# naturerobots/mesh_navigation

Measured on AMD Instinct MI355X. Metric: plans/sec (Dijkstra makePlan device path incl. computeVectorMap, 1M-vertex mesh), higher is better.
Workload: dtype f32

## Files before the change

### mesh_navigation_amd/csrc/mnav_tb_build.h

```cpp
#pragma once
#include <algorithm>
#include <cmath>
#include <cstdint>
#include <cstring>
#include <numeric>
#include <stdexcept>
#include <vector>

#include "mnav_build.h"

namespace mnav {

struct TbExp { uint32_t u, soff, sl, off; };

struct TbTile {
  uint32_t soff;
  uint32_t sl;
  uint32_t nv;
  uint32_t nh;
  uint32_t sweep_off;
  uint32_t sweep_chunks;
  uint32_t pre_off, pre_chunks;
  uint32_t post_off, post_chunks;
  uint32_t exp_off, exp_n;
  uint32_t v0;
  uint32_t goff;
  uint32_t ovf_off, ovf_n;
};
static_assert(sizeof(TbTile) == 64, "TbTile is read as one 64-byte scalar load");

constexpr uint32_t kTbChunk = 64;
constexpr uint32_t kTbBlock = 16;
constexpr uint32_t kTbBlocksPerChunk = 4;
constexpr uint32_t kTbGhostEdges = 5;
constexpr uint32_t kTbGhostEnd = 1u << 4;
constexpr uint32_t kTbTileEnd = 1u << 6;
constexpr uint32_t kTbOrderShift = 12;
constexpr uint32_t kTbInfBits = 0x7f800000u;
constexpr uint32_t kTbDirty = 0x80000000u;

constexpr uint32_t kTbFinSlots = 8;
constexpr uint16_t kTbFinNone = 0xFFFFu;
struct TbFinOvf { uint32_t y, src, wsrc, pad; };

struct TbvExp { uint32_t rows, soff, sl, off, n, pad[3]; };
static_assert(sizeof(TbvExp) == 32, "read as two 16-byte loads");

struct HostTb {
  std::vector<uint16_t> fin_src; std::vector<uint32_t> fin_wsrc; std::vector<TbFinOvf> fin_ovf;
  std::vector<uint32_t> ghost_gid;
  uint32_t T = 0, ntiles = 0, V = 0;
  uint64_t S = 0;
  uint32_t max_nh = 0, max_sl = 0;
  std::vector<TbTile> tiles;
  std::vector<uint32_t> stream;
  std::vector<uint32_t> wsrc;
  std::vector<uint32_t> vstream, vwsrc;
  std::vector<uint32_t> vtile;
  std::vector<TbvExp> vexps;
  std::vector<uint32_t> vgroups;
  std::vector<TbExp> exps;
  std::vector<uint32_t> verts;
  std::vector<uint32_t> vert_tile, vert_local;
};

namespace detail {
inline void tb_bisect(std::vector<uint32_t>& ids, size_t lo, size_t hi, size_t k, const float* xyz, uint32_t T, std::vector<uint32_t>& cuts)
{
  const size_t n = hi - lo;
  if (k <= 1) { cuts.push_back((uint32_t)hi); return; }
  float mn[3] = { INFINITY, INFINITY, INFINITY }, mx[3] = { -INFINITY, -INFINITY, -INFINITY };
  for (size_t i = lo; i < hi; ++i)
    for (int q = 0; q < 3; ++q) { const float x = xyz[3 * (size_t)ids[i] + q]; mn[q] = std::min(mn[q], x); mx[q] = std::max(mx[q], x); }
  int ax = 0;
  for (int q = 1; q < 3; ++q) if (mx[q] - mn[q] > mx[ax] - mn[ax]) ax = q;
  auto less = [&](uint32_t a, uint32_t b) {
    const float xa = xyz[3 * (size_t)a + ax], xb = xyz[3 * (size_t)b + ax];
    return xa < xb || (xa == xb && a < b);
  };
  int ax2 = (ax + 1) % 3;
  { const int o = (ax + 2) % 3; if (mx[o] - mn[o] > mx[ax2] - mn[ax2]) ax2 = o; }
  const size_t kl = k / 2, kr = k - kl;
  const size_t target = (size_t)((double)n * (double)kl / (double)k);
  const size_t f_lo = std::max<size_t>(n > kr * (size_t)T ? n - kr * (size_t)T : 1, 1), f_hi = std::min(kl * (size_t)T, n - 1);
  const size_t w = (size_t)(2.0 * std::sqrt((double)n)) + 8;
  const size_t a = target > w ? target - w : 0, b = std::min(target + w, n - 1);
  if (a > 0) std::nth_element(ids.begin() + lo, ids.begin() + lo + a, ids.begin() + hi, less);
  if (b + 1 < n) std::nth_element(ids.begin() + lo + a, ids.begin() + lo + b, ids.begin() + hi, less);
  std::sort(ids.begin() + lo + a, ids.begin() + lo + b + 1, less);
  auto gap_at = [&](size_t c) { return xyz[3 * (size_t)ids[lo + c] + ax] - xyz[3 * (size_t)ids[lo + c - 1] + ax]; };
  float maxgap = 0.f;
  for (size_t c = a + 1; c <= b; ++c) maxgap = std::max(maxgap, gap_at(c));
  const size_t c_lo = std::min(std::max(f_lo, a + 1), b), c_hi = std::max(std::min(f_hi, b), c_lo);
  size_t cut = std::min(std::max(target, c_lo), c_hi); float best = -1.f;
  for (size_t c = c_lo; c <= c_hi; ++c) {
    const float gap = gap_at(c);
    const size_t dc = c > target ? c - target : target - c, db = cut > target ? cut - target : target - cut;
    if (gap > best * 1.0001f + 1e-12f || (gap >= best && dc < db)) { best = gap; cut = c; }
  }
  if (best < 0.5f * maxgap) {
    cut = std::min(std::max(target, c_lo), c_hi);
    size_t rl = a, rr = b + 1;
    for (size_t c = cut; c > a; --c) if (gap_at(c) >= 0.5f * maxgap) { rl = c; break; }
    for (size_t c = cut + 1; c <= b; ++c) if (gap_at(c) >= 0.5f * maxgap) { rr = c; break; }
    std::sort(ids.begin() + lo + rl, ids.begin() + lo + rr, [&](uint32_t p, uint32_t q) {
      const float xp = xyz[3 * (size_t)p + ax2], xq = xyz[3 * (size_t)q + ax2];
      return xp < xq || (xp == xq && p < q);
    });
  }
  tb_bisect(ids, lo, lo + cut, kl, xyz, T, cuts);
  tb_bisect(ids, lo + cut, hi, kr, xyz, T, cuts);
}
}

inline void tb_div_magic(uint32_t d, uint32_t* magic, uint32_t* shift)
{
  if (d <= 1u) { *magic = 0u; *shift = 0u; return; }
  uint32_t s = 31u - (uint32_t)__builtin_clz(d);
  if ((d & (d - 1u)) == 0u) s -= 1u;
  *magic = (uint32_t)(((1ull << (32u + s)) + d - 1ull) / d); *shift = s;
}
inline uint32_t tb_div_by_magic(uint32_t n, uint32_t d, uint32_t magic, uint32_t shift)
{
  return d <= 1u ? n : ((uint32_t)(((uint64_t)n * magic) >> 32) >> shift);
}

inline uint32_t tb_sweep_index(uint32_t j, uint32_t q) { return 4u * q + j; }

constexpr uint32_t kTbvSources = 6;
constexpr uint32_t kTbvGhostRows = 64;
constexpr uint32_t kTbvSrc = 0x2000u, kTbvDst = 0xA000u;
constexpr uint32_t kTbvTileWords = 12;
constexpr uint32_t kTbvGhostEnd = 1u, kTbvTileEnd = 2u;
inline void tbv_set_source(uint32_t* blk, uint32_t k, uint32_t row)
{
  static const uint32_t dw[6] = { 0, 1, 1, 2, 2, 3 }, sh[6] = { 16, 0, 16, 0, 16, 0 };
  blk[dw[k]] = (blk[dw[k]] & ~(0xFFFFu << sh[k])) | ((kTbvSrc | row) << sh[k]);
}
inline void tbv_init_block(uint32_t* blk, uint32_t row, uint32_t mode = kTbvDst)
{
  for (uint32_t q = 0; q < kTbBlock; ++q) blk[q] = 0u;
  blk[0] = mode | row;
  for (uint32_t k = 0; k < kTbvSources; ++k) { tbv_set_source(blk, k, row); blk[8 + k] = 0x7f800000u; }
}
inline uint32_t tbv_target(const uint32_t* blk) { return blk[0] & 0xFFu; }
inline uint32_t tbv_flags(const uint32_t* blk) { return blk[3] >> 16; }
inline uint32_t tbv_source(const uint32_t* blk, uint32_t k)
{
  static const uint32_t dw[6] = { 0, 1, 1, 2, 2, 3 }, sh[6] = { 16, 0, 16, 0, 16, 0 };
  return (blk[dw[k]] >> sh[k]) & 0xFFu;
}
inline uint32_t tbv_append(std::vector<uint32_t>& stream, std::vector<uint32_t>& wsrc, std::vector<uint32_t>& blocks, std::vector<uint32_t>& bw,
                           uint32_t pad_row, uint32_t pad_mode, uint32_t min_chunks, uint32_t* chunks)
{
  const uint32_t first = (uint32_t)(stream.size() / kTbChunk);
  uint32_t n = (uint32_t)((blocks.size() / kTbBlock + kTbBlocksPerChunk - 1) / kTbBlocksPerChunk);
  n = std::max(n, min_chunks);
  while (blocks.size() < (size_t)n * kTbChunk) { const size_t at = blocks.size(); blocks.resize(at + kTbBlock); bw.resize(at + kTbBlock, 0xFFFFFFFFu); tbv_init_block(&blocks[at], pad_row, pad_mode); }
  for (uint32_t c = 0; c < n; ++c) {
    const size_t at = stream.size();
    stream.resize(at + kTbChunk); wsrc.resize(at + kTbChunk);
    for (uint32_t j = 0; j < kTbBlocksPerChunk; ++j)
      for (uint32_t q = 0; q < kTbBlock; ++q) {
        stream[at + tb_sweep_index(j, q)] = blocks[(size_t)c * kTbChunk + kTbBlock * j + q];
        wsrc[at + tb_sweep_index(j, q)] = bw[(size_t)c * kTbChunk + kTbBlock * j + q];
      }
  }
  *chunks = n;
  return first;
}

inline HostTb build_tb(const HostTopology& t, const float* xyz, uint32_t T)
{
  if (T == 0 || T > 255 || (T & 3)) throw std::invalid_argument("tile-batch engine: T must be a multiple of 4 below 256");
  HostTb H;
  const uint32_t V = t.V;
  H.T = T; H.V = V;
  H.verts.resize(V);
  std::iota(H.verts.begin(), H.verts.end(), 0u);
  std::vector<uint32_t> cuts;
  if (V) detail::tb_bisect(H.verts, 0, V, std::max<size_t>(1, (size_t)std::ceil((double)V / (0.9 * T))), xyz, T, cuts);
  H.ntiles = (uint32_t)cuts.size();
  H.vert_tile.assign(V, 0); H.vert_local.assign(V, 0);
  H.tiles.assign(H.ntiles, TbTile{});
  {
    uint32_t b = 0;
    for (uint32_t tl = 0; tl < H.ntiles; ++tl) {
      std::sort(H.verts.begin() + b, H.verts.begin() + cuts[tl]);
      H.tiles[tl].v0 = b; H.tiles[tl].nv = cuts[tl] - b;
      for (uint32_t i = b; i < cuts[tl]; ++i) { H.vert_tile[H.verts[i]] = tl; H.vert_local[H.verts[i]] = i - b; }
      b = cuts[tl];
    }
  }
  std::vector<std::vector<uint32_t>> ghosts(H.ntiles);
  auto gkey = [&](uint32_t v) { return ((uint64_t)H.vert_tile[v] << 32) | H.vert_local[v]; };
  for (uint32_t tl = 0; tl < H.ntiles; ++tl) {
    auto& g = ghosts[tl];
    const TbTile& L = H.tiles[tl];
    for (uint32_t i = 0; i < L.nv; ++i) {
      const uint32_t v = H.verts[L.v0 + i];
      for (uint32_t k = t.row_ptr[v]; k < t.row_ptr[v + 1]; ++k) if (H.vert_tile[t.nbr_u[k]] != tl) g.push_back(t.nbr_u[k]);
    }
    std::sort(g.begin(), g.end(), [&](uint32_t a, uint32_t b) { return gkey(a) < gkey(b); });
    g.erase(std::unique(g.begin(), g.end()), g.end());
    TbTile& W = H.tiles[tl];
    W.nh = (uint32_t)g.size();
    W.sl = T + ((W.nh + 3u) & ~3u);
    W.soff = (uint32_t)H.S;
    if (H.S + W.sl > 0xFFFFFFFFull) throw std::invalid_argument("tile-batch engine: mesh too large for 32-bit slice offsets");
    H.S += W.sl;
    H.max_nh = std::max(H.max_nh, W.nh); H.max_sl = std::max(H.max_sl, W.sl);
  }
  auto ghost_slot = [&](uint32_t tl, uint32_t v) -> uint32_t {
    const auto& g = ghosts[tl];
    const auto it = std::lower_bound(g.begin(), g.end(), v, [&](uint32_t a, uint32_t b) { return gkey(a) < gkey(b); });
    return (uint32_t)(it - g.begin());
  };
  H.fin_src.assign((size_t)H.ntiles * kTbFinSlots * T, kTbFinNone);
  H.fin_wsrc.assign((size_t)H.ntiles * kTbFinSlots * T, kNone);
  for (uint32_t tl = 0; tl < H.ntiles; ++tl) {
    TbTile& W = H.tiles[tl];
    W.goff = (uint32_t)H.ghost_gid.size();
    H.ghost_gid.insert(H.ghost_gid.end(), ghosts[tl].begin(), ghosts[tl].end());
    W.ovf_off = (uint32_t)H.fin_ovf.size();
    for (uint32_t y = 0; y < W.nv; ++y) {
      const uint32_t v = H.verts[W.v0 + y];
      uint32_t n = 0;
      for (uint32_t k = t.row_ptr[v]; k < t.row_ptr[v + 1]; ++k, ++n) {
        const uint32_t u = t.nbr_u[k];
        const uint32_t si = (H.vert_tile[u] == tl) ? H.vert_local[u] : T + ghost_slot(tl, u);
        if (si >= kTbFinNone) throw std::invalid_argument("tile-batch engine: a slice is too long for the finalize tables");
        if (n < kTbFinSlots) { const size_t at = ((size_t)tl * kTbFinSlots + n) * T + y; H.fin_src[at] = (uint16_t)si; H.fin_wsrc[at] = k; }
        else H.fin_ovf.push_back(TbFinOvf{ y, si, k, 0u });
      }
    }
    W.ovf_n = (uint32_t)H.fin_ovf.size() - W.ovf_off;
  }
  const uint32_t kRow = 256;
  uint32_t in_chunk = 0;
  uint32_t last_target = kNone;
  auto open_block = [&]() -> size_t {
    if (in_chunk == kTbBlocksPerChunk) { in_chunk = 0; last_target = kNone; }
    const size_t at = H.stream.size();
    H.stream.resize(at + kTbBlock, 0u); H.wsrc.resize(at + kTbBlock, kNone);
    ++in_chunk;
    return at;
  };
  auto chunk_prev = [&]() -> uint32_t { return (in_chunk == 0 || in_chunk == kTbBlocksPerChunk) ? kNone : last_target; };
  auto init_sweep_block = [&](size_t at, uint32_t row, uint32_t prev) {
    for (int q = 0; q <= 7; ++q) H.stream[at + q] = row * kRow;
    if (prev != kNone) H.stream[at + 1] = prev * kRow;
    for (int q = 8; q <= 14; ++q) H.stream[at + q] = kTbInfBits;
  };
  auto noop_sweep_block = [&]() {
    const uint32_t row = (last_target == 0u) ? 1u : 0u;
    const uint32_t prev = chunk_prev();
    const size_t at = open_block();
    init_sweep_block(at, row, prev);
    last_target = row;
  };
  auto close_chunk = [&](bool sweep) {
    if (in_chunk == 0) return;
    while (in_chunk < kTbBlocksPerChunk) { if (sweep) noop_sweep_block(); else open_block(); }
    in_chunk = 0; last_target = kNone;
  };
  std::vector<uint16_t> order;
  std::vector<std::pair<uint32_t, uint32_t>> srcs;
  std::vector<uint32_t> ts;
  for (uint32_t tl = 0; tl < H.ntiles; ++tl) {
    TbTile& W = H.tiles[tl];
    const auto& g = ghosts[tl];
    float mn[3] = { INFINITY, INFINITY, INFINITY }, mx[3] = { -INFINITY, -INFINITY, -INFINITY };
    for (uint32_t i = 0; i < W.nv; ++i)
      for (int k = 0; k < 3; ++k) { const float x = xyz[3 * (size_t)H.verts[W.v0 + i] + k]; mn[k] = std::min(mn[k], x); mx[k] = std::max(mx[k], x); }
    int a0 = 0, a1 = 1;
    {
      int idx[3] = { 0, 1, 2 };
      std::sort(idx, idx + 3, [&](int x, int y) { return (mx[x] - mn[x]) > (mx[y] - mn[y]) || ((mx[x] - mn[x]) == (mx[y] - mn[y]) && x < y); });
      a0 = std::min(idx[0], idx[1]); a1 = std::max(idx[0], idx[1]);
    }
    W.sweep_off = (uint32_t)(H.stream.size() / kTbChunk);
    static const float dirs[4][2] = { { 1, 1 }, { -1, 1 }, { -1, -1 }, { 1, -1 } };
    uint32_t order_chunks[4] = { 0, 0, 0, 0 };
    std::vector<uint32_t> vs[4], vw[4];
    for (int o = 0; o < 4; ++o) {
      order.resize(W.nv);
      for (uint32_t i = 0; i < W.nv; ++i) order[i] = (uint16_t)i;
      std::stable_sort(order.begin(), order.end(), [&](uint16_t x, uint16_t y) {
        const float* px = &xyz[3 * (size_t)H.verts[W.v0 + x]]; const float* py = &xyz[3 * (size_t)H.verts[W.v0 + y]];
        return dirs[o][0] * px[a0] + dirs[o][1] * px[a1] < dirs[o][0] * py[a0] + dirs[o][1] * py[a1];
      });
      for (uint32_t i = 0; i < W.nv; ++i) {
        const uint32_t y = order[i], v = H.verts[W.v0 + y];
        uint32_t k6 = kTbvSources; size_t at = 0;
        for (uint32_t k = t.row_ptr[v]; k < t.row_ptr[v + 1]; ++k) {
          if (H.vert_tile[t.nbr_u[k]] != tl) continue;
          if (k6 == kTbvSources) { at = vs[o].size(); vs[o].resize(at + kTbBlock); vw[o].resize(at + kTbBlock, kNone); tbv_init_block(&vs[o][at], kTbvGhostRows + y); k6 = 0; }
          tbv_set_source(&vs[o][at], k6, kTbvGhostRows + H.vert_local[t.nbr_u[k]]); vw[o][at + 8 + k6] = k; ++k6;
        }
      }
      const size_t first = H.stream.size() / kTbChunk;
      for (uint32_t i = 0; i < W.nv; ++i) {
        const uint32_t y = order[i], v = H.verts[W.v0 + y];
        srcs.clear();
        for (uint32_t k = t.row_ptr[v]; k < t.row_ptr[v + 1]; ++k)
          if (H.vert_tile[t.nbr_u[k]] == tl) srcs.push_back({ H.vert_local[t.nbr_u[k]], k });
        while (!srcs.empty()) {
          if (chunk_prev() == y) noop_sweep_block();
          const uint32_t prev = chunk_prev();
          const size_t at = open_block();
          init_sweep_block(at, y, prev);
          last_target = y;
          uint32_t slot = 1;
          if (prev != kNone) {
            for (size_t e = 0; e < srcs.size(); ++e)
              if (srcs[e].first == prev) { H.wsrc[at + 8] = srcs[e].second; srcs.erase(srcs.begin() + e); break; }
            slot = 2;
          }
          while (slot <= 7 && !srcs.empty()) {
            H.stream[at + slot] = srcs.front().first * kRow; H.wsrc[at + 7 + slot] = srcs.front().second;
            srcs.erase(srcs.begin()); ++slot;
          }
        }
      }
      close_chunk(true);
      order_chunks[o] = (uint32_t)(H.stream.size() / kTbChunk - first);
    }
    W.sweep_chunks = std::max(std::max(order_chunks[0], order_chunks[1]), std::max(order_chunks[2], order_chunks[3]));
    {
      std::vector<uint32_t> st2, ws2;
      size_t src = (size_t)W.sweep_off * kTbChunk;
      for (int o = 0; o < 4; ++o) {
        const size_t len = (size_t)order_chunks[o] * kTbChunk;
        st2.insert(st2.end(), H.stream.begin() + src, H.stream.begin() + src + len);
        ws2.insert(ws2.end(), H.wsrc.begin() + src, H.wsrc.begin() + src + len);
        src += len;
        for (uint32_t c = order_chunks[o]; c < W.sweep_chunks; ++c)
          for (uint32_t j = 0; j < kTbBlocksPerChunk; ++j) {
            const size_t at = st2.size();
            st2.resize(at + kTbBlock, 0u); ws2.resize(at + kTbBlock, kNone);
            for (int q = 0; q <= 7; ++q) st2[at + q] = (j & 1u) * kRow;
            if (j) st2[at + 1] = ((j - 1u) & 1u) * kRow;
            for (int q = 8; q <= 14; ++q) st2[at + q] = kTbInfBits;
          }
      }
      H.stream.resize((size_t)W.sweep_off * kTbChunk); H.wsrc.resize((size_t)W.sweep_off * kTbChunk);
      H.stream.insert(H.stream.end(), st2.begin(), st2.end()); H.wsrc.insert(H.wsrc.end(), ws2.begin(), ws2.end());
    }
    for (size_t c = (size_t)W.sweep_off; c < (size_t)W.sweep_off + 4u * W.sweep_chunks; ++c)
      for (uint32_t j = 1; j < kTbBlocksPerChunk; ++j) {
        const uint32_t* K = &H.stream[c * kTbChunk + kTbBlock * j];
        const uint32_t* Ws = &H.wsrc[c * kTbChunk + kTbBlock * j];
        const uint32_t prev = K[-(int)kTbBlock];
        bool ok = K[0] != prev && K[1] == prev;
        for (int q = 2; q <= 7; ++q) ok = ok && !(K[q] == prev && Ws[7 + q] != kNone);
        if (!ok) throw std::logic_error("tile-batch streams: a follower block breaks the forwarding rules");
      }
    for (size_t c = (size_t)W.sweep_off; c < (size_t)W.sweep_off + 4u * W.sweep_chunks; ++c) {
      uint32_t tmp[kTbChunk], tmpw[kTbChunk];
      std::copy(H.stream.begin() + c * kTbChunk, H.stream.begin() + (c + 1) * kTbChunk, tmp);
      std::copy(H.wsrc.begin() + c * kTbChunk, H.wsrc.begin() + (c + 1) * kTbChunk, tmpw);
      for (uint32_t j = 0; j < kTbBlocksPerChunk; ++j)
        for (uint32_t q = 0; q < kTbBlock; ++q) {
          H.stream[c * kTbChunk + tb_sweep_index(j, q)] = tmp[kTbBlock * j + q];
          H.wsrc[c * kTbChunk + tb_sweep_index(j, q)] = tmpw[kTbBlock * j + q];
        }
    }
    uint32_t v_sweep_off = 0, v_sweep_chunks = 0;
    {
      size_t vblocks = 0;
      for (int o = 0; o < 4; ++o) vblocks = std::max(vblocks, vs[o].size() / kTbBlock);
      const uint32_t vchunks = (uint32_t)((vblocks + kTbBlocksPerChunk - 1) / kTbBlocksPerChunk);
      for (int o = 0; o < 4; ++o) {
        uint32_t n = 0;
        const uint32_t first = tbv_append(H.vstream, H.vwsrc, vs[o], vw[o], kTbvGhostRows, kTbvDst, vchunks, &n);
        if (o == 0) { v_sweep_off = first; v_sweep_chunks = n; }
      }
    }
    float cen[2] = { 0.f, 0.f };
    for (uint32_t i = 0; i < W.nv; ++i) { const float* q = &xyz[3 * (size_t)H.verts[W.v0 + i]]; cen[0] += q[a0]; cen[1] += q[a1]; }
    if (W.nv) { cen[0] /= (float)W.nv; cen[1] /= (float)W.nv; }
    auto ghost_order = [&](uint32_t gv) -> uint32_t {
// ... 129 lines not shown
```

### mesh_navigation_amd/csrc/mnav_tb_finalize.h

```cpp
#pragma once

namespace {

typedef float f32x3_u __attribute__((ext_vector_type(3), aligned(4)));

struct FinRec { float* dist; uint32_t* pred; float* vm; uint32_t seed; float cut; uint32_t tie; uint32_t pad_[3]; };
static_assert(sizeof(FinRec) == 48, "FinRec: 12 dwords");
constexpr uint32_t kFinRecWords = 12;

struct FinTb {
  const uint16_t* src; const float* w; const TbFinOvf* ovf; const float* ovf_w;
  const uint32_t* verts; const uint32_t* ghost_gid; const uint32_t* order;
  const float* xyz; float* const* vecmaps;
  const Plan* plans; PlanResult* res; uint32_t* mismatch; const FinRec* recs;
  uint32_t plans_per_wave, tiles_per_xcd, max_sl;
};

__global__ __launch_bounds__(kBlock) void k_tb_fin_plans(tb::Args A, const Plan* __restrict__ plans, float* const* __restrict__ vecmaps, FinRec* __restrict__ recs)
{
  const uint32_t p = blockIdx.x * kBlock + threadIdx.x;
  if (p >= A.NP) return;
  const Plan& P = plans[p];
  const float dt = A.D[tb::slot_addr(A.vaddr[A.target[p]], A.NP, p)];
  const GoalCut gc = goal_cut(dt, A.offset, A.target[p]);
  Ctl r; memset(&r, 0, sizeof(r));
  r.armed = dt < inf_f() ? 1u : 0u; r.goal_dist = gc.goal; r.thr = inf_f(); r.thr_fixed = inf_f();
  r.it = (int32_t)A.ctl->iters; r.done = 1u; r.overflow = (A.ctl->err || A.ctl->n_cand[0]) ? 1u : 0u;
  P.ctl[0] = r; P.ctl[1] = r;
  FinRec fr; memset(&fr, 0, sizeof(fr));
  fr.dist = P.dist; fr.pred = P.pred; fr.vm = vecmaps ? vecmaps[p] : nullptr; fr.seed = A.seed[p]; fr.cut = gc.cut; fr.tie = gc.tie;
  recs[p] = fr;
}

__global__ __launch_bounds__(kBlock) void k_tb_fin_weights(size_t n, const uint32_t* __restrict__ wsrc, const Nbr* __restrict__ nbr, float* __restrict__ w)
{
  const size_t stride = (size_t)gridDim.x * kBlock;
  for (size_t i = (size_t)blockIdx.x * kBlock + threadIdx.x; i < n; i += stride) w[i] = (wsrc[i] == kNone) ? inf_f() : nbr[wsrc[i]].w;
}

#ifndef MNAV_FIN_WAVES
#define MNAV_FIN_WAVES 4
#endif
#ifndef MNAV_FIN_OCC
#define MNAV_FIN_OCC 3
#endif
constexpr int kFinWaves = MNAV_FIN_WAVES;
#ifndef MNAV_FIN_NOTAB
constexpr uint32_t kFinTabSlots = 6;
#else
constexpr uint32_t kFinTabSlots = 0;
#endif
constexpr uint32_t kFinTabRows = 128, kFinTabWords = 3 * kFinTabSlots * kFinTabRows, kFinNoSlot = 255;
__host__ __device__ constexpr uint32_t fin_lds_words(uint32_t max_sl, bool vecmap) { return 5u * max_sl + (vecmap ? kFinTabWords : 0u); }
template <int T>
__global__ __launch_bounds__(64 * kFinWaves, MNAV_FIN_OCC) void k_tb_finalize(tb::Args A, FinTb F)
{
  extern __shared__ __attribute__((aligned(16))) uint32_t fin_lds_all[];
  const int lane = threadIdx.x & 63, wave = threadIdx.x >> 6;
  uint32_t* const fin_lds = fin_lds_all + (size_t)wave * fin_lds_words(F.max_sl, F.vecmaps != nullptr);
  float* const ltab = reinterpret_cast<float*>(fin_lds + 5u * F.max_sl);
  const uint32_t xcd = blockIdx.x & 7u, j = blockIdx.x >> 3;
  const uint32_t grp = xcd * F.tiles_per_xcd + j % F.tiles_per_xcd, pg = j / F.tiles_per_xcd;
  const uint32_t t_raw = grp * kFinWaves + wave;
  const bool live = t_raw < A.ntiles;
#ifdef MNAV_FIN_BISECTION_ORDER
  const uint32_t t = live ? t_raw : A.ntiles - 1u;
#else
  const uint32_t t = F.order[live ? t_raw : A.ntiles - 1u];
#endif
  const uint32_t p_beg = pg * F.plans_per_wave, p_end = min(p_beg + F.plans_per_wave, A.NP);
  if (grp * kFinWaves >= A.ntiles || p_beg >= p_end) return;
  const TbTile W = A.tiles[t];
  uint32_t* const ld = fin_lds;
  uint32_t* const lgid = fin_lds + F.max_sl;
  float* const lxyz = reinterpret_cast<float*>(fin_lds + 2 * F.max_sl);
  const uint32_t NP = A.NP;
  for (uint32_t i = lane; i < W.sl; i += 64) {
    uint32_t g = kNone;
    if (i < W.nv) g = F.verts[W.v0 + i];
    else if (i >= (uint32_t)T && i - T < W.nh) g = F.ghost_gid[W.goff + (i - T)];
    lgid[i] = g;
    if (F.vecmaps && g != kNone) { lxyz[3 * i] = F.xyz[3 * (size_t)g]; lxyz[3 * i + 1] = F.xyz[3 * (size_t)g + 1]; lxyz[3 * i + 2] = F.xyz[3 * (size_t)g + 2]; }
  }
  uint32_t ys[2] = { (uint32_t)lane, (uint32_t)lane + 64u };
  bool own[2]; uint32_t gid[2];
  uint32_t src[2][kTbFinSlots], srck[2][kTbFinSlots]; float wt[2][kTbFinSlots];
#pragma unroll
  for (int v = 0; v < 2; ++v) {
    own[v] = live && ys[v] < W.nv;
#pragma unroll
    for (int k = 0; k < (int)kTbFinSlots; ++k) {
      const size_t at = ((size_t)t * kTbFinSlots + k) * T + (own[v] ? ys[v] : 0u);
      src[v][k] = own[v] ? (uint32_t)F.src[at] : (uint32_t)kTbFinNone;
      wt[v][k] = own[v] ? F.w[at] : inf_f();
    }
  }
  __builtin_amdgcn_wave_barrier();
#pragma unroll
  for (int v = 0; v < 2; ++v) {
    gid[v] = own[v] ? lgid[ys[v]] : kNone;
#ifdef MNAV_FIN_TILEMAJOR_EXPERIMENT
    if (own[v]) gid[v] = min(t * (uint32_t)T + ys[v], 999999u);
#endif
#pragma unroll
    for (int k = 0; k < (int)kTbFinSlots; ++k)
      if (src[v][k] == kTbFinNone) src[v][k] = ys[v] < (uint32_t)T ? ys[v] : 0u;
#pragma unroll
    for (int k = 0; k < (int)kTbFinSlots; ++k) srck[v][k] = src[v][k] | ((uint32_t)k << 16);
  }
  float px[2] = { 0.f, 0.f }, py[2] = { 0.f, 0.f }, pz[2] = { 0.f, 0.f };
  if (F.vecmaps) {
#pragma unroll
    for (int v = 0; v < 2; ++v) if (own[v]) { px[v] = lxyz[3 * ys[v]]; py[v] = lxyz[3 * ys[v] + 1]; pz[v] = lxyz[3 * ys[v] + 2]; }
#pragma unroll
    for (int v = 0; v < 2; ++v) if (own[v]) {
#pragma unroll
      for (int k = 0; k < (int)kFinTabSlots; ++k) {
        const uint32_t sx = src[v][k];
        float x = lxyz[3 * sx] - px[v], y = lxyz[3 * sx + 1] - py[v], z = lxyz[3 * sx + 2] - pz[v];
        const float len = sqrtf(x * x + y * y + z * z);
        x = x / len; y = y / len; z = z / len;
        float* const tp = ltab + (uint32_t)k * kFinTabRows + ys[v];
        tp[0] = x; tp[kFinTabSlots * kFinTabRows] = y; tp[2 * kFinTabSlots * kFinTabRows] = z;
      }
    }
  }
  MNAV_GLOBAL const float* const gD = as_global(A.D) + (size_t)W.soff * NP;
  const uint32_t i0 = lane, i1 = lane + 64u, i2 = lane + 128u, i3 = lane + 192u;
  const uint32_t slm = W.sl - 1u, j0 = min(i0, slm), j1 = min(i1, slm), j2 = min(i2, slm), j3 = min(i3, slm);
  MNAV_GLOBAL const uint32_t* const g_recs = (MNAV_GLOBAL const uint32_t*)as_global(F.recs) + min((uint32_t)lane, kFinRecWords - 1u);
  auto load_slice = [&](uint32_t p, uint32_t& rec, uint32_t (&r)[4]) {
    MNAV_GLOBAL const uint32_t* s = (MNAV_GLOBAL const uint32_t*)(gD + (size_t)p * W.sl);
    rec = g_recs[(size_t)p * kFinRecWords];
    r[0] = s[j0]; r[1] = s[j1]; r[2] = s[j2]; r[3] = s[j3];
  };
  uint32_t cur[4], nxt[4], rcur, rnxt;
  load_slice(p_beg, rcur, cur);
  rnxt = rcur;
  uint32_t bad = 0;
  for (uint32_t p = p_beg; p < p_end; ++p) {
#ifndef MNAV_FIN_NOSYNC
    __syncthreads();
#endif
    if (p + 1 < p_end) load_slice(p + 1, rnxt, nxt);
    auto rw = [&](int k) { return (uint32_t)__builtin_amdgcn_readlane((int)rcur, k); };
    MNAV_GLOBAL float* const g_dist = (MNAV_GLOBAL float*)(uintptr_t)(((unsigned long long)rw(1) << 32) | rw(0));
    MNAV_GLOBAL uint32_t* const g_pred = (MNAV_GLOBAL uint32_t*)(uintptr_t)(((unsigned long long)rw(3) << 32) | rw(2));
    MNAV_GLOBAL float* const g_vm = (MNAV_GLOBAL float*)(uintptr_t)(((unsigned long long)rw(5) << 32) | rw(4));
    const uint32_t seed = rw(6);
    const bool reached = __ballot(cur[0] != kTbInfBits || cur[1] != kTbInfBits || cur[2] != kTbInfBits || cur[3] != kTbInfBits) != 0ull;
    uint32_t cnt = 0;
    if (!reached) {
#pragma unroll
      for (int v = 0; v < 2; ++v) if (own[v]) {
        g_dist[gid[v]] = inf_f(); g_pred[gid[v]] = gid[v];
        if (g_vm) { const f32x3_u z3 = { 0.f, 0.f, 0.f }; *(MNAV_GLOBAL f32x3_u*)(g_vm + 3 * (size_t)gid[v]) = z3; }
      }
    } else {
      GoalCut gcut; gcut.goal = 0.f; gcut.cut = u2f(rw(7)); gcut.tie = rw(8);
      __builtin_amdgcn_wave_barrier();
      if (i0 < W.sl) ld[i0] = cur[0];
      if (i1 < W.sl) ld[i1] = cur[1];
      if (i2 < W.sl) ld[i2] = cur[2];
      if (i3 < W.sl) ld[i3] = cur[3];
      for (uint32_t i = lane + 256u; i < W.sl; i += 64) ld[i] = ((MNAV_GLOBAL const uint32_t*)(gD + (size_t)p * W.sl))[i];
      __builtin_amdgcn_wave_barrier();
#pragma unroll
      for (int v = 0; v < 2; ++v) {
        const uint32_t dyb = ld[ys[v]];
        const float dy = u2f(dyb);
        uint32_t sum[kTbFinSlots], dsb[kTbFinSlots];
        bool at_cut = false;
#pragma unroll
        for (int k = 0; k < (int)kTbFinSlots; ++k) {
          dsb[k] = ld[src[v][k]];
          const float ds = u2f(dsb[k]);
          at_cut |= ds == gcut.cut;
          sum[k] = (ds < gcut.cut) ? f2u(ds + wt[v][k]) : kTbInfBits;
        }
        const uint32_t m = min(min(min(sum[0], sum[1]), min(sum[2], sum[3])), min(min(sum[4], sum[5]), min(sum[6], sum[7])));
        const bool is_seed = gid[v] == seed;
        const bool cut = dy > gcut.cut;
        uint32_t val = cut ? m : dyb;
        uint32_t c[kTbFinSlots];
#pragma unroll
        for (int k = 0; k < (int)kTbFinSlots; ++k) c[k] = (sum[k] == val) ? dsb[k] : kTbInfBits;
        const uint32_t bd = min(min(min(c[0], c[1]), min(c[2], c[3])), min(min(c[4], c[5]), min(c[6], c[7])));
        uint32_t best = ys[v] | (kFinNoSlot << 16), nbest = 0;
#pragma unroll
        for (int k = (int)kTbFinSlots - 1; k >= 0; --k) { const bool hit = c[k] == bd; best = hit ? srck[v][k] : best; nbest += hit ? 1u : 0u; }
        uint32_t best_s = best & 0xFFFFu, bk = best >> 16;
        const bool finite = val != kTbInfBits;
        unsigned long long key = finite && bd != kTbInfBits ? (((unsigned long long)bd << 32) | lgid[best_s]) : ~0ull;
        uint32_t nbad = (m < val && !is_seed) ? 1u : 0u;
        if (own[v] && (at_cut || (finite && nbest > 1u) || W.ovf_n)) {
          nbad = 0u;
#pragma unroll
          for (int k = 0; k < (int)kTbFinSlots; ++k) {
            const float ds = u2f(dsb[k]);
            bool ex = ds < inf_f() && ds < gcut.cut;
            if (ds == gcut.cut && ds < inf_f()) ex = lgid[src[v][k]] < gcut.tie;
            sum[k] = ex ? f2u(ds + wt[v][k]) : kTbInfBits;
          }
          val = cut ? kTbInfBits : dyb;
          if (cut) {
#pragma unroll
            for (int k = 0; k < (int)kTbFinSlots; ++k) val = min(val, sum[k]);
          }
          key = ~0ull; best_s = ys[v]; bk = kFinNoSlot;
#pragma unroll
          for (int k = 0; k < (int)kTbFinSlots; ++k) {
            if (sum[k] < val && !is_seed) ++nbad;
            if (sum[k] == val && val != kTbInfBits) {
              const unsigned long long kk = ((unsigned long long)dsb[k] << 32) | lgid[src[v][k]];
              if (kk < key) { key = kk; best_s = src[v][k]; }
            }
          }
          for (uint32_t e = 0; e < W.ovf_n; ++e) {
            const TbFinOvf o = F.ovf[W.ovf_off + e];
            if (o.y != ys[v]) continue;
            const uint32_t db = ld[o.src], g2 = lgid[o.src];
            if (!expanded_source(gcut, u2f(db), g2)) continue;
            const uint32_t sm = f2u(u2f(db) + F.ovf_w[W.ovf_off + e]);
            if (cut && sm < val) { val = sm; key = ~0ull; }
            else if (sm < val && !is_seed) ++nbad;
            if (sm == val && val != kTbInfBits) {
              const unsigned long long kk = ((unsigned long long)db << 32) | g2;
              if (kk < key) { key = kk; best_s = o.src; }
            }
          }
        }
        if (!own[v]) continue;
        bad += nbad;
        uint32_t pv = gid[v];
        float outd = u2f(val);
        if (is_seed) { outd = dy; ++cnt; }
        else {
          if (val != kTbInfBits && key == ~0ull) ++bad;
          if (val != kTbInfBits) { pv = (uint32_t)key; ++cnt; }
        }
#ifdef MNAV_FIN_NOSTORE
        if (MNAV_FIN_NOSTORE == 1) { bad += (f2u(outd) ^ pv) == 0x12345u ? 1u : 0u; }
        else { g_dist[gid[v]] = outd; g_pred[gid[v]] = pv; }
#else
        g_dist[gid[v]] = outd; g_pred[gid[v]] = pv;
#endif
        if (g_vm) {
          float x = 0.f, y = 0.f, z = 0.f;
          if (pv != gid[v]) {
            if (bk < kFinTabSlots) {
              const float* const tp = ltab + bk * kFinTabRows + ys[v];
              x = tp[0]; y = tp[kFinTabSlots * kFinTabRows]; z = tp[2 * kFinTabSlots * kFinTabRows];
            } else {
              x = lxyz[3 * best_s] - px[v]; y = lxyz[3 * best_s + 1] - py[v]; z = lxyz[3 * best_s + 2] - pz[v];
              const float len = sqrtf(x * x + y * y + z * z);
              x = x / len; y = y / len; z = z / len;
            }
          }
          const f32x3_u o3 = { x, y, z };
#ifdef MNAV_FIN_NOSTORE
          bad += (f2u(x) ^ f2u(y) ^ f2u(z)) == 0x12345u ? 1u : 0u;
#else
          *(MNAV_GLOBAL f32x3_u*)(g_vm + 3 * (size_t)gid[v]) = o3;
#endif
        }
      }
    }
    cnt = wave_sum(cnt);
    if (lane == 0 && cnt && live) atomicAdd(&F.res[p].settled, (unsigned long long)cnt);
#pragma unroll
    for (int q = 0; q < 4; ++q) cur[q] = nxt[q];
    rcur = rnxt;
  }
  bad = wave_sum(bad);
  if (lane == 0 && bad) atomicAdd(F.mismatch, bad);
}

}
```

Before: 41160.

## Specialize finalize loop by slot count and interior tiles, batch settled counts

The finalize kernel now checks per block whether any vertex uses neighbor slots 6 or 7 and instantiates the plan loop for 6 or 8 slots. A separate interior-tile path skips the cut comparisons. The host sorts each vertex's neighbors by id so the tie-break matches and the exact fallback runs less often. Settled counts are gathered per lane and written with one atomic per 64 plans, and the double-buffered slice loads avoid register copies. This adds code size and register pressure, plus an extra block-level barrier for the width vote.

```diff
diff --git a/mesh_navigation_amd/csrc/mnav_tb_build.h b/mesh_navigation_amd/csrc/mnav_tb_build.h
--- a/mesh_navigation_amd/csrc/mnav_tb_build.h
+++ b/mesh_navigation_amd/csrc/mnav_tb_build.h
@@ -5,6 +5,7 @@
 #include <cstring>
 #include <numeric>
 #include <stdexcept>
+#include <utility>
 #include <vector>
 
 #include "mnav_build.h"
@@ -218,6 +219,7 @@
   };
   H.fin_src.assign((size_t)H.ntiles * kTbFinSlots * T, kTbFinNone);
   H.fin_wsrc.assign((size_t)H.ntiles * kTbFinSlots * T, kNone);
+  std::vector<std::pair<uint32_t, uint32_t>> fin_by_id;
   for (uint32_t tl = 0; tl < H.ntiles; ++tl) {
     TbTile& W = H.tiles[tl];
     W.goff = (uint32_t)H.ghost_gid.size();
@@ -225,9 +227,11 @@
     W.ovf_off = (uint32_t)H.fin_ovf.size();
     for (uint32_t y = 0; y < W.nv; ++y) {
       const uint32_t v = H.verts[W.v0 + y];
-      uint32_t n = 0;
-      for (uint32_t k = t.row_ptr[v]; k < t.row_ptr[v + 1]; ++k, ++n) {
-        const uint32_t u = t.nbr_u[k];
+      fin_by_id.clear();
+      for (uint32_t k = t.row_ptr[v]; k < t.row_ptr[v + 1]; ++k) fin_by_id.emplace_back(t.nbr_u[k], k);
+      std::sort(fin_by_id.begin(), fin_by_id.end());
+      for (uint32_t n = 0; n < (uint32_t)fin_by_id.size(); ++n) {
+        const uint32_t u = fin_by_id[n].first, k = fin_by_id[n].second;
         const uint32_t si = (H.vert_tile[u] == tl) ? H.vert_local[u] : T + ghost_slot(tl, u);
         if (si >= kTbFinNone) throw std::invalid_argument("tile-batch engine: a slice is too long for the finalize tables");
         if (n < kTbFinSlots) { const size_t at = ((size_t)tl * kTbFinSlots + n) * T + y; H.fin_src[at] = (uint16_t)si; H.fin_wsrc[at] = k; }
diff --git a/mesh_navigation_amd/csrc/mnav_tb_finalize.h b/mesh_navigation_amd/csrc/mnav_tb_finalize.h
--- a/mesh_navigation_amd/csrc/mnav_tb_finalize.h
+++ b/mesh_navigation_amd/csrc/mnav_tb_finalize.h
@@ -56,7 +56,7 @@
 __global__ __launch_bounds__(64 * kFinWaves, MNAV_FIN_OCC) void k_tb_finalize(tb::Args A, FinTb F)
 {
   extern __shared__ __attribute__((aligned(16))) uint32_t fin_lds_all[];
-  const int lane = threadIdx.x & 63, wave = threadIdx.x >> 6;
+  const int lane = threadIdx.x & 63, wave = __builtin_amdgcn_readfirstlane(threadIdx.x >> 6);
   uint32_t* const fin_lds = fin_lds_all + (size_t)wave * fin_lds_words(F.max_sl, F.vecmaps != nullptr);
   float* const ltab = reinterpret_cast<float*>(fin_lds + 5u * F.max_sl);
   const uint32_t xcd = blockIdx.x & 7u, j = blockIdx.x >> 3;
@@ -95,6 +95,7 @@
       wt[v][k] = own[v] ? F.w[at] : inf_f();
     }
   }
+  const bool wide_tile = W.ovf_n != 0u || __ballot(src[0][6] != kTbFinNone || src[0][7] != kTbFinNone || src[1][6] != kTbFinNone || src[1][7] != kTbFinNone) != 0ull;
   __builtin_amdgcn_wave_barrier();
 #pragma unroll
   for (int v = 0; v < 2; ++v) {
@@ -108,16 +109,14 @@
 #pragma unroll
     for (int k = 0; k < (int)kTbFinSlots; ++k) srck[v][k] = src[v][k] | ((uint32_t)k << 16);
   }
-  float px[2] = { 0.f, 0.f }, py[2] = { 0.f, 0.f }, pz[2] = { 0.f, 0.f };
   if (F.vecmaps) {
 #pragma unroll
-    for (int v = 0; v < 2; ++v) if (own[v]) { px[v] = lxyz[3 * ys[v]]; py[v] = lxyz[3 * ys[v] + 1]; pz[v] = lxyz[3 * ys[v] + 2]; }
-#pragma unroll
     for (int v = 0; v < 2; ++v) if (own[v]) {
+      const float px = lxyz[3 * ys[v]], py = lxyz[3 * ys[v] + 1], pz = lxyz[3 * ys[v] + 2];
 #pragma unroll
       for (int k = 0; k < (int)kFinTabSlots; ++k) {
         const uint32_t sx = src[v][k];
-        float x = lxyz[3 * sx] - px[v], y = lxyz[3 * sx + 1] - py[v], z = lxyz[3 * sx + 2] - pz[v];
+        float x = lxyz[3 * sx] - px, y = lxyz[3 * sx + 1] - py, z = lxyz[3 * sx + 2] - pz;
         const float len = sqrtf(x * x + y * y + z * z);
         x = x / len; y = y / len; z = z / len;
         float* const tp = ltab + (uint32_t)k * kFinTabRows + ys[v];
@@ -129,149 +128,207 @@
   const uint32_t i0 = lane, i1 = lane + 64u, i2 = lane + 128u, i3 = lane + 192u;
   const uint32_t slm = W.sl - 1u, j0 = min(i0, slm), j1 = min(i1, slm), j2 = min(i2, slm), j3 = min(i3, slm);
   MNAV_GLOBAL const uint32_t* const g_recs = (MNAV_GLOBAL const uint32_t*)as_global(F.recs) + min((uint32_t)lane, kFinRecWords - 1u);
-  auto load_slice = [&](uint32_t p, uint32_t& rec, uint32_t (&r)[4]) {
+  auto load_slice = [&](uint32_t p, uint32_t& rec, uint32_t (&r)[4]) __attribute__((always_inline)) {
     MNAV_GLOBAL const uint32_t* s = (MNAV_GLOBAL const uint32_t*)(gD + (size_t)p * W.sl);
     rec = g_recs[(size_t)p * kFinRecWords];
     r[0] = s[j0]; r[1] = s[j1]; r[2] = s[j2]; r[3] = s[j3];
   };
-  uint32_t cur[4], nxt[4], rcur, rnxt;
-  load_slice(p_beg, rcur, cur);
-  rnxt = rcur;
+  static_assert(kTbFinSlots == 8, "the plan loop is instantiated for 6 and 8 slots");
+  if (lane == 0) ld[0] = wide_tile ? 1u : 0u;
+  __syncthreads();
+  bool wide = false;
+#pragma unroll
+  for (int w = 0; w < kFinWaves; ++w) wide |= fin_lds_all[(size_t)w * fin_lds_words(F.max_sl, F.vecmaps != nullptr)] != 0u;
+  __syncthreads();
   uint32_t bad = 0;
-  for (uint32_t p = p_beg; p < p_end; ++p) {
+  struct FinV { uint32_t dyb, val, best, pvk, nbad; bool has, cutv, is_seed, need; };
+  auto plan_loop = [&](auto ns_tag) __attribute__((always_inline)) {
+    constexpr int NS = decltype(ns_tag)::value;
+    uint32_t settled = 0;
+    auto step = [&](uint32_t p, uint32_t (&cur)[4], uint32_t rcur, uint32_t (&nxt)[4], uint32_t& rnxt) __attribute__((always_inline)) {
 #ifndef MNAV_FIN_NOSYNC
-    __syncthreads();
-#endif
-    if (p + 1 < p_end) load_slice(p + 1, rnxt, nxt);
-    auto rw = [&](int k) { return (uint32_t)__builtin_amdgcn_readlane((int)rcur, k); };
-    MNAV_GLOBAL float* const g_dist = (MNAV_GLOBAL float*)(uintptr_t)(((unsigned long long)rw(1) << 32) | rw(0));
-    MNAV_GLOBAL uint32_t* const g_pred = (MNAV_GLOBAL uint32_t*)(uintptr_t)(((unsigned long long)rw(3) << 32) | rw(2));
-    MNAV_GLOBAL float* const g_vm = (MNAV_GLOBAL float*)(uintptr_t)(((unsigned long long)rw(5) << 32) | rw(4));
-    const uint32_t seed = rw(6);
-    const bool reached = __ballot(cur[0] != kTbInfBits || cur[1] != kTbInfBits || cur[2] != kTbInfBits || cur[3] != kTbInfBits) != 0ull;
-    uint32_t cnt = 0;
-    if (!reached) {
-#pragma unroll
-      for (int v = 0; v < 2; ++v) if (own[v]) {
-        g_dist[gid[v]] = inf_f(); g_pred[gid[v]] = gid[v];
-        if (g_vm) { const f32x3_u z3 = { 0.f, 0.f, 0.f }; *(MNAV_GLOBAL f32x3_u*)(g_vm + 3 * (size_t)gid[v]) = z3; }
-      }
-    } else {
-      GoalCut gcut; gcut.goal = 0.f; gcut.cut = u2f(rw(7)); gcut.tie = rw(8);
-      __builtin_amdgcn_wave_barrier();
-      if (i0 < W.sl) ld[i0] = cur[0];
-      if (i1 < W.sl) ld[i1] = cur[1];
-      if (i2 < W.sl) ld[i2] = cur[2];
-      if (i3 < W.sl) ld[i3] = cur[3];
-      for (uint32_t i = lane + 256u; i < W.sl; i += 64) ld[i] = ((MNAV_GLOBAL const uint32_t*)(gD + (size_t)p * W.sl))[i];
-      __builtin_amdgcn_wave_barrier();
-#pragma unroll
-      for (int v = 0; v < 2; ++v) {
-        const uint32_t dyb = ld[ys[v]];
-        const float dy = u2f(dyb);
-        uint32_t sum[kTbFinSlots], dsb[kTbFinSlots];
-        bool at_cut = false;
-#pragma unroll
-        for (int k = 0; k < (int)kTbFinSlots; ++k) {
-          dsb[k] = ld[src[v][k]];
-          const float ds = u2f(dsb[k]);
-          at_cut |= ds == gcut.cut;
-          sum[k] = (ds < gcut.cut) ? f2u(ds + wt[v][k]) : kTbInfBits;
+      __syncthreads();
+#endif
+      load_slice(min(p + 1u, p_end - 1u), rnxt, nxt);
+      auto rw = [&](int k) { return (uint32_t)__builtin_amdgcn_readlane((int)rcur, k); };
+      MNAV_GLOBAL float* const g_dist = (MNAV_GLOBAL float*)(uintptr_t)(((unsigned long long)rw(1) << 32) | rw(0));
+      MNAV_GLOBAL uint32_t* const g_pred = (MNAV_GLOBAL uint32_t*)(uintptr_t)(((unsigned long long)rw(3) << 32) | rw(2));
+      MNAV_GLOBAL float* const g_vm = (MNAV_GLOBAL float*)(uintptr_t)(((unsigned long long)rw(5) << 32) | rw(4));
+      const uint32_t seed = rw(6);
+      const bool reached = __ballot(cur[0] != kTbInfBits || cur[1] != kTbInfBits || cur[2] != kTbInfBits || cur[3] != kTbInfBits) != 0ull;
+      bool counted[2] = { false, false };
+      if (!reached) {
+#pragma unroll
+        for (int v = 0; v < 2; ++v) if (own[v]) {
+          g_dist[gid[v]] = inf_f(); g_pred[gid[v]] = gid[v];
+          if (g_vm) { const f32x3_u z3 = { 0.f, 0.f, 0.f }; *(MNAV_GLOBAL f32x3_u*)(g_vm + 3 * (size_t)gid[v]) = z3; }
         }
-        const uint32_t m = min(min(min(sum[0], sum[1]), min(sum[2], sum[3])), min(min(sum[4], sum[5]), min(sum[6], sum[7])));
-        const bool is_seed = gid[v] == seed;
-        const bool cut = dy > gcut.cut;
-        uint32_t val = cut ? m : dyb;
-        uint32_t c[kTbFinSlots];
-#pragma unroll
-        for (int k = 0; k < (int)kTbFinSlots; ++k) c[k] = (sum[k] == val) ? dsb[k] : kTbInfBits;
-        const uint32_t bd = min(min(min(c[0], c[1]), min(c[2], c[3])), min(min(c[4], c[5]), min(c[6], c[7])));
-        uint32_t best = ys[v] | (kFinNoSlot << 16), nbest = 0;
-#pragma unroll
-        for (int k = (int)kTbFinSlots - 1; k >= 0; --k) { const bool hit = c[k] == bd; best = hit ? srck[v][k] : best; nbest += hit ? 1u : 0u; }
-        uint32_t best_s = best & 0xFFFFu, bk = best >> 16;
-        const bool finite = val != kTbInfBits;
-        unsigned long long key = finite && bd != kTbInfBits ? (((unsigned long long)bd << 32) | lgid[best_s]) : ~0ull;
-        uint32_t nbad = (m < val && !is_seed) ? 1u : 0u;
-        if (own[v] && (at_cut || (finite && nbest > 1u) || W.ovf_n)) {
-          nbad = 0u;
-#pragma unroll
-          for (int k = 0; k < (int)kTbFinSlots; ++k) {
+      } else {
+        const uint32_t cutb = rw(7);
+        GoalCut gcut; gcut.goal = 0.f; gcut.cut = u2f(cutb); gcut.tie = rw(8);
+        __builtin_amdgcn_wave_barrier();
+        ld[j0] = cur[0]; ld[j1] = cur[1]; ld[j2] = cur[2]; ld[j3] = cur[3];
+        for (uint32_t i = lane + 256u; i < W.sl; i += 64) ld[i] = ((MNAV_GLOBAL const uint32_t*)(gD + (size_t)p * W.sl))[i];
+        __builtin_amdgcn_wave_barrier();
+        auto common = [&](const int v, auto interior_tag, FinV& o) __attribute__((always_inline)) {
+          constexpr bool INTERIOR = decltype(interior_tag)::value;
+          const uint32_t dyb = cur[v];
+          const float dy = u2f(dyb);
+          uint32_t sum[NS], dsb[NS];
+          bool at_cut = false;
+#pragma unroll
+          for (int k = 0; k < NS; ++k) {
+            dsb[k] = ld[src[v][k]];
+            const float ds = u2f(dsb[k]);
+            if (INTERIOR) sum[k] = f2u(ds + wt[v][k]);
+            else {
+              at_cut |= ds == gcut.cut;
+              sum[k] = (ds < gcut.cut) ? f2u(ds + wt[v][k]) : kTbInfBits;
+            }
+          }
+          uint32_t m = sum[0];
+#pragma unroll
+          for (int k = 1; k < NS; ++k) m = min(m, sum[k]);
+          o.is_seed = gid[v] == seed;
+          o.cutv = dy > gcut.cut;
+          o.dyb = dyb;
+          o.val = o.cutv ? m : dyb;
+          uint32_t c[NS];
+#pragma unroll
+          for (int k = 0; k < NS; ++k) c[k] = (sum[k] == o.val) ? dsb[k] : kTbInfBits;
+          uint32_t bd = c[0];
+#pragma unroll
+          for (int k = 1; k < NS; ++k) bd = min(bd, c[k]);
+          uint32_t best = ys[v] | (kFinNoSlot << 16);
+#pragma unroll
+          for (int k = NS - 1; k >= 0; --k) best = (c[k] == bd) ? srck[v][k] : best;
+          o.best = best;
+          const bool finite = o.val != kTbInfBits;
+          o.has = finite && bd != kTbInfBits;
+          const uint32_t best_gid = lgid[best & 0xFFFFu];
+          o.pvk = o.has ? best_gid : ~0u;
+          o.nbad = (m < o.val && !o.is_seed) ? 1u : 0u;
+          o.need = !INTERIOR && own[v] && (at_cut || W.ovf_n);
+        };
+        auto exact = [&](const int v, FinV& o) __attribute__((always_inline)) {
+          uint32_t sum[NS], dsb[NS];
+          uint32_t nbad = 0u;
+          auto src_gid = [&](int k) __attribute__((always_inline)) { uint32_t s = src[v][k]; asm volatile("" : "+v"(s)); return lgid[s]; };
+#pragma unroll
+          for (int k = 0; k < NS; ++k) {
+            dsb[k] = ld[src[v][k]];
             const float ds = u2f(dsb[k]);
             bool ex = ds < inf_f() && ds < gcut.cut;
-            if (ds == gcut.cut && ds < inf_f()) ex = lgid[src[v][k]] < gcut.tie;
+            if (ds == gcut.cut && ds < inf_f()) ex = src_gid(k) < gcut.tie;
             sum[k] = ex ? f2u(ds + wt[v][k]) : kTbInfBits;
           }
-          val = cut ? kTbInfBits : dyb;
-          if (cut) {
-#pragma unroll
-            for (int k = 0; k < (int)kTbFinSlots; ++k) val = min(val, sum[k]);
-          }
-          key = ~0ull; best_s = ys[v]; bk = kFinNoSlot;
-#pragma unroll
-          for (int k = 0; k < (int)kTbFinSlots; ++k) {
-            if (sum[k] < val && !is_seed) ++nbad;
+          uint32_t val = o.cutv ? kTbInfBits : o.dyb;
+          if (o.cutv) {
+#pragma unroll
+            for (int k = 0; k < NS; ++k) val = min(val, sum[k]);
+          }
+          unsigned long long key = ~0ull;
+          uint32_t best_s = ys[v];
+#pragma unroll
+          for (int k = 0; k < NS; ++k) {
+            if (sum[k] < val && !o.is_seed) ++nbad;
             if (sum[k] == val && val != kTbInfBits) {
-              const unsigned long long kk = ((unsigned long long)dsb[k] << 32) | lgid[src[v][k]];
+              const unsigned long long kk = ((unsigned long long)dsb[k] << 32) | src_gid(k);
               if (kk < key) { key = kk; best_s = src[v][k]; }
             }
           }
           for (uint32_t e = 0; e < W.ovf_n; ++e) {
-            const TbFinOvf o = F.ovf[W.ovf_off + e];
-            if (o.y != ys[v]) continue;
-            const uint32_t db = ld[o.src], g2 = lgid[o.src];
+            const TbFinOvf ov = F.ovf[W.ovf_off + e];
+            if (ov.y != ys[v]) continue;
+            const uint32_t db = ld[ov.src], g2 = lgid[ov.src];
             if (!expanded_source(gcut, u2f(db), g2)) continue;
             const uint32_t sm = f2u(u2f(db) + F.ovf_w[W.ovf_off + e]);
-            if (cut && sm < val) { val = sm; key = ~0ull; }
-            else if (sm < val && !is_seed) ++nbad;
+            if (o.cutv && sm < val) { val = sm; key = ~0ull; }
+            else if (sm < val && !o.is_seed) ++nbad;
             if (sm == val && val != kTbInfBits) {
               const unsigned long long kk = ((unsigned long long)db << 32) | g2;
-              if (kk < key) { key = kk; best_s = o.src; }
-            }
-          }
-        }
-        if (!own[v]) continue;
-        bad += nbad;
-        uint32_t pv = gid[v];
-        float outd = u2f(val);
-        if (is_seed) { outd = dy; ++cnt; }
-        else {
-          if (val != kTbInfBits && key == ~0ull) ++bad;
-          if (val != kTbInfBits) { pv = (uint32_t)key; ++cnt; }
-        }
+              if (kk < key) { key = kk; best_s = ov.src; }
+            }
+          }
+          o.val = val; o.nbad = nbad; o.best = best_s | (kFinNoSlot << 16); o.has = key != ~0ull; o.pvk = (uint32_t)key;
+        };
+        auto store = [&](const int v, const FinV& o) __attribute__((always_inline)) {
+          const bool fin = o.val != kTbInfBits, use = fin && !o.is_seed;
+          const uint32_t pv = use ? o.pvk : gid[v];
+          const float outd = u2f(o.is_seed ? o.dyb : o.val);
+          const uint32_t best_s = o.best & 0xFFFFu, bk = o.best >> 16;
+          const bool moves = pv != gid[v];
+          float x = 0.f, y = 0.f, z = 0.f;
+          if (g_vm && kFinTabSlots > 0u) {
+            const float* const tp = ltab + min(bk, kFinTabSlots - 1u) * kFinTabRows + ys[v];
+            const float tx = tp[0], ty = tp[kFinTabSlots * kFinTabRows], tz = tp[2 * kFinTabSlots * kFinTabRows];
+            const bool tab = moves && bk < kFinTabSlots;
+            x = tab ? tx : 0.f; y = tab ? ty : 0.f; z = tab ? tz : 0.f;
+          }
+          if (!own[v]) return;
+          bad += o.nbad + ((use && !o.has) ? 1u : 0u);
+          counted[v] = fin || o.is_seed;
 #ifdef MNAV_FIN_NOSTORE
-        if (MNAV_FIN_NOSTORE == 1) { bad += (f2u(outd) ^ pv) == 0x12345u ? 1u : 0u; }
-        else { g_dist[gid[v]] = outd; g_pred[gid[v]] = pv; }
+          if (MNAV_FIN_NOSTORE == 1) { bad += (f2u(outd) ^ pv) == 0x12345u ? 1u : 0u; }
+          else { g_dist[gid[v]] = outd; g_pred[gid[v]] = pv; }
 #else
-        g_dist[gid[v]] = outd; g_pred[gid[v]] = pv;
-#endif
-        if (g_vm) {
-          float x = 0.f, y = 0.f, z = 0.f;
-          if (pv != gid[v]) {
-            if (bk < kFinTabSlots) {
-              const float* const tp = ltab + bk * kFinTabRows + ys[v];
-              x = tp[0]; y = tp[kFinTabSlots * kFinTabRows]; z = tp[2 * kFinTabSlots * kFinTabRows];
-            } else {
-              x = lxyz[3 * best_s] - px[v]; y = lxyz[3 * best_s + 1] - py[v]; z = lxyz[3 * best_s + 2] - pz[v];
+          g_dist[gid[v]] = outd; g_pred[gid[v]] = pv;
+#endif
+          if (g_vm) {
+            if (moves && bk >= kFinTabSlots) {
+              x = lxyz[3 * best_s] - lxyz[3 * ys[v]]; y = lxyz[3 * best_s + 1] - lxyz[3 * ys[v] + 1]; z = lxyz[3 * best_s + 2] - lxyz[3 * ys[v] + 2];
               const float len = sqrtf(x * x + y * y + z * z);
               x = x / len; y = y / len; z = z / len;
             }
-          }
-          const f32x3_u o3 = { x, y, z };
+            const f32x3_u o3 = { x, y, z };
 #ifdef MNAV_FIN_NOSTORE
-          bad += (f2u(x) ^ f2u(y) ^ f2u(z)) == 0x12345u ? 1u : 0u;
+            bad += (f2u(x) ^ f2u(y) ^ f2u(z)) == 0x12345u ? 1u : 0u;
 #else
-          *(MNAV_GLOBAL f32x3_u*)(g_vm + 3 * (size_t)gid[v]) = o3;
-#endif
-        }
+            *(MNAV_GLOBAL f32x3_u*)(g_vm + 3 * (size_t)gid[v]) = o3;
+#endif
+          }
+        };
+        auto body = [&](auto interior_tag) __attribute__((always_inline)) {
+          FinV r0, r1;
+          if (NS <= 6) {
+            common(0, interior_tag, r0); common(1, interior_tag, r1);
+            if (__ballot(r0.need || r1.need) != 0ull) {
+              if (r0.need) exact(0, r0);
+              if (r1.need) exact(1, r1);
+            }
+            store(0, r0); store(1, r1);
+          } else {
+            common(0, interior_tag, r0); if (r0.need) exact(0, r0); store(0, r0);
+            common(1, interior_tag, r1); if (r1.need) exact(1, r1); store(1, r1);
+          }
+        };
+        bool outside = false;
+#pragma unroll
+        for (int q = 0; q < 4; ++q) outside |= !(u2f(cur[q]) < gcut.cut || (cur[q] == kTbInfBits && cutb != kTbInfBits));
+        const bool interior = W.sl <= 256u && W.ovf_n == 0u && __ballot(outside) == 0ull;
+        if (interior) body(std::true_type{});
+        else body(std::false_type{});
       }
+      const uint32_t cnt = (uint32_t)__popcll(__ballot(counted[0])) + (uint32_t)__popcll(__ballot(counted[1]));
+      const uint32_t q = (p - p_beg) & 63u;
+      settled += (uint32_t)lane == q ? cnt : 0u;
+      if (q == 63u || p + 1u == p_end) {
+        const uint32_t pl = p - q + (uint32_t)lane;
+        if (settled && pl < p_end) atomicAdd(&F.res[pl].settled, (unsigned long long)settled);
+        settled = 0;
+      }
+    };
+    uint32_t sa[4], sb[4], ra, rb;
+    load_slice(p_beg, ra, sa);
+    rb = ra;
+    for (uint32_t p = p_beg; p < p_end; p += 2) {
+      step(p, sa, ra, sb, rb);
+      if (p + 1u >= p_end) break;
+      step(p + 1u, sb, rb, sa, ra);
     }
-    cnt = wave_sum(cnt);
-    if (lane == 0 && cnt && live) atomicAdd(&F.res[p].settled, (unsigned long long)cnt);
-#pragma unroll
-    for (int q = 0; q < 4; ++q) cur[q] = nxt[q];
-    rcur = rnxt;
-  }
+  };
+  if (wide) plan_loop(std::integral_constant<int, 8>{});
+  else plan_loop(std::integral_constant<int, 6>{});
   bad = wave_sum(bad);
   if (lane == 0 && bad) atomicAdd(F.mismatch, bad);
 }
```

New measurement: 41500 (median of 6 runs). Within noise of the previous version (+0.8%).
